# liangheming/simple_pose

Hardware: AMD Instinct MI355X
Metric: images/sec fwd+decode, ResNet50-DConv 256x192 bs=128 (higher is better)
Workload: dtype f32; 1 GPU; ResNet50-DConv 256x192 bs=128 per GPU, fp32 forward (NCHW in -> heat maps) + GaussTaylor decode, eval-mode BN, conditioned random weights; images_per_gpu=128, global_batch=128, parallelism=replicas x1 (no collective), ranks=1 process(es), one per GPU, launch=stream launches, tile_table=profiles/r06_dconv_f32_tiles.json, batches_in_flight=2, decode=in line, HSA_ENABLE_IPC_MODE_LEGACY=0

## Files before the change

include/simple_pose_hip.h:

```cpp
#ifndef SIMPLE_POSE_HIP_H
#define SIMPLE_POSE_HIP_H

#include <stdint.h>

#ifdef __cplusplus
extern "C" {
#endif

#define SP_OK 0
#define SP_EINVAL (-1)
#define SP_ELAUNCH (-2)

#define SP_ABI_VERSION 36

#define SP_CONV_RELU 0x1u
#define SP_CONV_OUT_NCHW 0x2u
#define SP_CONV_PIXEL_SHUFFLE 0x4u
#define SP_CONV_OUT_F32 0x10u
#define SP_CONV_BN_Y_MASK 0x20u
#define SP_CONV_BF16 0x8u
#define SP_CONV_HARDSWISH 0x40u
#define SP_CONV_OUT_SLICE 0x80u

typedef struct sp_conv_desc {
// ... 20 lines not shown
#define SP_CONV_KERNEL_RING_LW 3
#define SP_CONV_KERNEL_RING_LW4 4
#define SP_CONV_KERNEL_PW 2

int sp_abi_version(void);
const char* sp_last_error(void);


int sp_nchw_to_nhwc4(const float* x_nchw, float* y_nhwc4, int batch, int channels, int h, int w, void* stream);

int sp_conv2d_fwd(const sp_conv_desc* desc, const void* x, const void* w_packed, const float* scale,
                  const float* shift, const void* residual, void* y, void* stream);

int sp_conv3x3_direct_ok(const sp_conv_desc* desc);
int sp_conv3x3_direct(const sp_conv_desc* desc, const void* x, const void* w_packed, const float* scale, const float* shift,
                      const void* residual, void* y, void* stream);

int sp_basic_block_c32_ok(const sp_conv_desc* desc);
int sp_basic_block_c32(const sp_conv_desc* desc, const void* x, const void* w1_packed, const float* scale1, const float* shift1,
                       const void* w2_packed, const float* scale2, const float* shift2, void* y, void* stream);

int sp_basic_block_c64_ok(const sp_conv_desc* desc);
int sp_basic_block_c64(const sp_conv_desc* desc, const void* x, const void* w1_packed, const float* scale1, const float* shift1,
                       const void* w2_packed, const float* scale2, const float* shift2, void* y, void* stream);

int sp_dual_pw_bf16_ok(int64_t rows, int c_main, int c_short, int c_out);
int sp_dual_pw_f32_ok(int64_t rows, int c_main, int c_short, int c_out);
int sp_dual_pw_f32(const float* a_main, const float* w_main_packed, const float* scale_main, const float* shift_main, const float* a_short,
                   const float* w_short_packed, const float* scale_short, const float* shift_short, float* y, int64_t rows, int c_main, int c_short,
                   int c_out, int relu, void* stream);
int sp_dual_pw_bf16(const void* a_main, const void* w_main_packed, const float* scale_main, const float* shift_main, const void* a_short,
                    const void* w_short_packed, const float* scale_short, const float* shift_short, void* y, int64_t rows, int c_main, int c_short,
                    int c_out, int relu, void* stream);
int sp_bottleneck_c64_ok(const sp_conv_desc* desc);
int sp_bottleneck_c64(const sp_conv_desc* desc, const void* x, const void* w1_packed, const float* scale1, const float* shift1,
                      const void* w2_packed, const float* scale2, const float* shift2, const void* w3_packed, const float* scale3,
                      const float* shift3, void* y, void* stream);

int sp_stem7_pool_ok(int batch, int h, int w);
int sp_stem7_pool(const float* x, const void* w_packed, int k_pad, const float* scale, const float* shift, void* y, int bf16,
                  int batch, int h, int w, void* stream);
int sp_stem7_pool_u8(const unsigned char* crops_bgr, const float* mean_rgb_host, const void* w_packed, int k_pad, const float* scale,
                     const float* shift, void* y, int bf16, int batch, int h, int w, void* stream);

int sp_hrnet_transition1_ok(int c_in, int h, int w);
int sp_hrnet_transition1(const void* x, int batch, int h, int w, const void* wa_packed, int k_pad, const float* scale_a, const float* shift_a,
                         const void* wb_packed, const float* scale_b, const float* shift_b, void* y_hi, void* y_lo, void* stream);
int sp_hrnet_stem_ok(int batch, int h, int w);
int sp_hrnet_stem(const float* x, const void* w1_packed, int k1_pad, const float* scale1, const float* shift1, const void* w2_packed,
                  const float* scale2, const float* shift2, void* y, int batch, int h, int w, void* stream);

int sp_conv2d_pw_ok(const sp_conv_desc* desc);

int sp_conv2d_ring_ok(const sp_conv_desc* desc);

int sp_conv2d_kernel_name(const sp_conv_desc* desc, int has_residual, int variant, char* buf, int cap);

int sp_conv2d_default_tile(const sp_conv_desc* desc, int* tile_m, int* tile_n);

int sp_maxpool3x3s2_nhwc(const float* x, float* y, int batch, int h, int w, int c, void* stream);

int sp_pixel_shuffle2_nhwc(const float* x, float* y, int batch, int h, int w, int c, void* stream);

int sp_global_avg_pool_nhwc(const float* x, float* y, int batch, int hw, int c, void* stream);
int sp_se_gate_add_relu_nhwc(const float* x, const float* gate_logits, const float* identity, float* y, int batch, int hw,
                             int c, void* stream);
// ... 321 lines not shown
```

simple_pose_amd/_lib.py:

```python
from __future__ import annotations

import ctypes
import os
from ctypes import c_double, c_float, c_int, c_int32, c_int64, c_uint32, c_void_p

from .build import LIB_PATH as _DEFAULT_LIB_PATH

LIB_PATH = os.environ.get("SIMPLE_POSE_HIP_LIB", _DEFAULT_LIB_PATH)

SP_CONV_RELU = 0x1
SP_CONV_OUT_NCHW = 0x2
SP_CONV_PIXEL_SHUFFLE = 0x4
SP_CONV_BF16 = 0x8
SP_CONV_OUT_F32 = 0x10
SP_CONV_BN_Y_MASK = 0x20
SP_CONV_HARDSWISH = 0x40
SP_CONV_OUT_SLICE = 0x80
SP_LETTERBOX_FOCUS, SP_LETTERBOX_U8 = 0, 1
SP_YOLO_NMS_MAX_CANDIDATES, SP_YOLO_NMS_MAX_DET = 32768, 1024
SP_COCO_MAX_JOINTS, SP_COCO_MAX_GT_PER_IMAGE, SP_COCO_MAX_DT_PER_IMAGE, SP_COCO_MAX_DETS = 64, 128, 2048, 32
SP_COCO_DT_XY_F64, SP_COCO_DT_SCORE_F64, SP_COCO_GT_CROWD, SP_COCO_GT_IGNORE = 1, 2, 1, 2
CONV_TILES =((128, 128), (64, 128), (128, 64), (64, 64), (256, 64), (128, 32))
ABI_VERSION = 36
SP_CONV_KERNEL_IGEMM, SP_CONV_KERNEL_RING, SP_CONV_KERNEL_PW, SP_CONV_KERNEL_RING_LW, SP_CONV_KERNEL_RING_LW4 = 0, 1, 2, 3, 4
# ... 116 lines not shown
    "sp_coco_kp_accumulate": (c_int, [_P, _P, _P, _P, _P, c_int, c_int, c_int, c_int, c_int, ctypes.POINTER(c_double), c_int, _P, c_int64, _P, _P, _P]),
    "sp_pixel_unshuffle2_nhwc": (c_int, [_P, _P, c_int, c_int, c_int, c_int, _P]),
    "sp_pixel_unshuffle2_nhwc_bf16": (c_int, [_P, _P, c_int, c_int, c_int, c_int, _P]),
    "sp_maxpool3x3s2_idx_nhwc": (c_int, [_P, c_int, _P, _P, c_int, c_int, c_int, c_int, _P]),
    "sp_maxpool3x3s2_bwd_idx_nhwc": (c_int, [_P, _P, c_int, _P, c_int, c_int, c_int, c_int, _P]),
    "sp_nchw_to_nhwc_pad": (c_int, [_P, _P, c_int, c_int, c_int, c_int, c_int, c_int, _P]),
    "sp_warp_affine_u8c3": (c_int, [_P, c_int, c_int, _P, c_int, _P, c_int, c_int, _P]),
    "sp_warp_affine_batch_u8c3_to_nchw_f32": (c_int, [_P, _P, _P, _P, c_int, c_int, c_int, ctypes.POINTER(c_float), _P, _P, _P]),
    "sp_conv2d_bn_stats_rows": (c_int, [ctypes.POINTER(ConvDesc), ctypes.POINTER(c_int)]),
    "sp_conv2d_fwd_bn_stats": (c_int, [ctypes.POINTER(ConvDesc), _P, _P, _P, _P, _P, c_int, _P]),
    "sp_conv2d_fwd_bn_stats_abn": (c_int, [ctypes.POINTER(ConvDesc), _P, _P, _P, _P, _P, _P, _P, _P, _P, _P, _P, c_int, _P]),
    "sp_bn_train_stats_from_conv": (c_int, [_P, _P, c_int, c_int, c_int64, c_int, c_float, c_float, _P, _P, _P, _P, _P]),
    "sp_conv2d_dgrad_bn_bwd_stats": (c_int, [ctypes.POINTER(ConvDesc), _P, _P, _P, _P, _P, _P, _P, _P, _P, _P, c_int, _P]),
    "sp_conv2d_dgrad_bn_bwd_stats2": (c_int, [ctypes.POINTER(ConvDesc), _P, _P, _P, _P, _P, _P, _P, _P, _P, _P, _P, _P, _P, _P, c_int, _P]),
    "sp_conv2d_dgrad_bn_bwd_stats_macc": (c_int, [ctypes.POINTER(ConvDesc), _P, _P, _P, _P, _P, _P, _P, _P, _P, _P, _P, _P, _P, _P, _P, c_int, _P]),
    "sp_conv2d_dgrad_phases": (c_int, [ctypes.POINTER(ConvDesc), c_int, _P, ctypes.POINTER(_P), _P, _P, _P, _P, _P, _P, _P, _P, _P, _P, _P, _P, c_int, _P]),
    "sp_bn_sums_from_conv": (c_int, [_P, _P, c_int, c_int, c_int, _P, _P]),
    "sp_bn_fold_apply_nhwc": (c_int, [_P, c_int, _P, _P, c_int, c_int, c_int64, c_float, c_float, _P, _P, _P, _P, c_int64, c_int, c_int, _P, _P, _P, _P, _P, _P]),
    "sp_bn_fold_bwd_apply_nhwc": (c_int, [_P, c_int, _P, _P, _P, _P, _P, c_int, c_int, _P, _P, _P, c_int64, c_int64, c_int, _P, _P, _P, _P, _P, _P, c_int, _P]),
    "sp_bn_bwd_sums_from_conv": (c_int, [_P, _P, c_int, c_int, c_int, _P, _P, _P]),
    "sp_bn_bwd_sums_from_conv_pair": (c_int, [_P, _P, _P, c_int, c_int, c_int, _P, _P, _P, _P, _P]),
    "sp_u8hwc_bgr_to_nhwc": (c_int, [_P, _P, c_int, c_int, c_int, c_int, _P, _P]),
    "sp_nchw_to_nhwc4_bf16": (c_int, [_P, _P, c_int, c_int, c_int, c_int, _P]),
    "sp_conv3x3_direct_ok": (c_int, [ctypes.POINTER(ConvDesc)]),
    "sp_conv3x3_direct": (c_int, [ctypes.POINTER(ConvDesc), _P, _P, _P, _P, _P, _P, _P]),
    "sp_basic_block_c32_ok": (c_int, [ctypes.POINTER(ConvDesc)]),
    "sp_basic_block_c32": (c_int, [ctypes.POINTER(ConvDesc), _P, _P, _P, _P, _P, _P, _P, _P, _P]),
    "sp_basic_block_c64_ok": (c_int, [ctypes.POINTER(ConvDesc)]),
    "sp_basic_block_c64": (c_int, [ctypes.POINTER(ConvDesc), _P, _P, _P, _P, _P, _P, _P, _P, _P]),
    "sp_dual_pw_bf16_ok": (c_int, [c_int64, c_int, c_int, c_int]),
    "sp_dual_pw_f32_ok": (c_int, [c_int64, c_int, c_int, c_int]),
    "sp_dual_pw_f32": (c_int, [_P, _P, _P, _P, _P, _P, _P, _P, _P, c_int64, c_int, c_int, c_int, c_int, _P]),
    "sp_dual_pw_bf16": (c_int, [_P, _P, _P, _P, _P, _P, _P, _P, _P, c_int64, c_int, c_int, c_int, c_int, _P]),
    "sp_bottleneck_c64_ok": (c_int, [ctypes.POINTER(ConvDesc)]),
    "sp_conv2d_pw_ok": (c_int, [ctypes.POINTER(ConvDesc)]),
    "sp_hrnet_stem_ok": (c_int, [c_int, c_int, c_int]),
    "sp_hrnet_stem": (c_int, [_P, _P, c_int, _P, _P, _P, _P, _P, _P, c_int, c_int, c_int, _P]),
    "sp_hrnet_transition1_ok": (c_int, [c_int, c_int, c_int]),
    "sp_hrnet_transition1": (c_int, [_P, c_int, c_int, c_int, _P, c_int, _P, _P, _P, _P, _P, _P, _P, _P]),
    "sp_stem7_pool_ok": (c_int, [c_int, c_int, c_int]),
    "sp_stem7_pool": (c_int, [_P, _P, c_int, _P, _P, _P, c_int, c_int, c_int, c_int, _P]),
    "sp_stem7_pool_u8": (c_int, [_P, ctypes.POINTER(ctypes.c_float), _P, c_int, _P, _P, _P, c_int, c_int, c_int, c_int, _P]),
    "sp_bottleneck_c64": (c_int, [ctypes.POINTER(ConvDesc), _P, _P, _P, _P, _P, _P, _P, _P, _P, _P, _P, _P]),
    "sp_masked_mse": (c_int, [_P, _P, _P, c_int, c_int, c_int, _P, _P, _P, _P]),
    "sp_conv_packed_dims": (c_int, [c_int, c_int, c_int, ctypes.POINTER(c_int), ctypes.POINTER(c_int)]),
    "sp_pack_conv_weights": (c_int, [_P, c_int, c_int, c_int, c_int, c_int, c_int, c_int, c_int, c_int, c_int, _P, c_int, _P]),
    "sp_pack_conv_weights_grouped": (c_int, [_P, c_int, c_int, c_int, c_int, c_int, _P, c_int, _P]),
    "sp_pack_conv_weights_grouped_taps": (c_int, [_P, c_int, c_int, c_int, c_int, c_int, c_int, c_int, c_int, c_int, c_int, c_int, c_int, _P, c_int, _P]),
    "sp_conv2d_wgrad_grouped_workspace": (c_int, [c_int, c_int, c_int, c_int, c_int, c_int, ctypes.POINTER(c_int64)]),
    "sp_conv2d_wgrad_grouped": (c_int, [_P, _P, c_int, c_int, c_int, c_int, c_int, c_int, c_int, c_int, c_int, c_int, c_int, c_int, _P, _P, c_int64, _P]),
    "sp_pack_deconv_k4s2p1": (c_int, [_P, c_int, c_int, c_int, _P, c_int, _P]),
    "sp_fold_bn": (c_int, [_P, _P, _P, _P, c_int, c_float, c_int, _P, _P, _P]),
    "sp_yolo_letterbox": (c_int, [_P, c_int, c_int, c_int, c_int, c_int, c_int, c_int, c_int, c_int, c_int, _P, _P]),
    "sp_yolo_focus_nchw": (c_int, [_P, c_int, c_int, c_int, _P, _P]),
    "sp_yolo_spp_nhwc": (c_int, [_P, c_int, c_int, c_int, c_int, c_int, _P]),
    "sp_upsample2_slice_nhwc": (c_int, [_P, c_int, _P, c_int, c_int, c_int, c_int, c_int, _P]),
    "sp_yolo_head_decode": (c_int, [_P, _P, _P, c_int, ctypes.POINTER(c_int32), c_int, c_int, c_int, ctypes.POINTER(c_float), ctypes.POINTER(c_float), _P, _P]),
    "sp_yolo_nms_workspace": (c_int, [c_int, ctypes.POINTER(c_int64)]),
    "sp_yolo_nms": (c_int, [_P, c_int, c_int, c_int, c_float, c_float, c_int, c_int, c_int, c_int, _P, c_int64, _P, ctypes.POINTER(c_int32), ctypes.POINTER(c_int32), _P]),
    "sp_yolo_boxes_to_source": (c_int, [_P, c_int, c_float, c_float, c_float, c_float, c_float, _P]),
    "sp_yolo_nms_device": (c_int, [_P, c_int, c_int, c_int, c_float, c_float, c_int, c_int, c_int, c_int, _P, c_int64, _P, _P, _P, _P]),
    "sp_topdown_plan": (c_int, [_P, _P, c_int, c_int, c_int, c_float, c_int, c_int, c_int, c_int, c_int, _P, _P, _P, _P, _P, _P, _P, _P, _P, _P, _P]),
    "sp_warp_affine_plan_u8c3": (c_int, [_P, c_int, c_int, c_int, _P, _P, _P, c_int, _P, c_int, c_int, _P]),
    "sp_mirror_w": (c_int, [_P, _P, c_int64, c_int, c_int, _P]),
    "sp_heat_map_flip_merge": (c_int, [_P, _P, ctypes.POINTER(c_int32), c_int, c_int, c_int, c_int, c_int, _P, _P]),
    "sp_track_associate": (c_int, [_P, _P, _P, _P, _P, _P, c_int, c_int, ctypes.POINTER(c_double), c_double, c_int, c_int, _P, _P, _P, _P, _P, _P, _P, _P,
# ... 102 lines not shown
```

simple_pose_amd/csrc/conv_pw.hip:

```cpp
#include "sp_common.h"

namespace {

struct PwArgs {
    const float* x;
    const float* w;
    const float* scale;
    const float* shift;
    const float* res;
    float* y;
    int M, N, nchunks, tiles_m, relu;
    unsigned x_bytes, y_bytes;
};

constexpr int BM = 64;
constexpr int TRS = 68;
constexpr unsigned OOB = 0x80000000u;

template <int K>
__global__ __launch_bounds__(256, 1) void conv_pw_kernel(const PwArgs p) {
    constexpr int CH = K / 4;
    constexpr int NG = K / 8;
    constexpr int APT = BM * CH / 256;
    extern __shared__ __align__(16) float smem[];
// ... 210 lines not shown
                    for (int i = 0; i < 2; ++i) fa[(g + 1) & 1][i] = *reinterpret_cast<const f32x4*>(a + swz(i * 32 + fr, 2 * (g + 1) + fh));
                }
#pragma unroll
                for (int s = 0; s < 4; ++s)
#pragma unroll
                    for (int i = 0; i < 2; ++i)
#pragma unroll
                        for (int n = 0; n < 2; ++n)
                            acc[q][i][n] = __builtin_amdgcn_mfma_f32_32x32x2f32(fa[g & 1][i][s], fb[q][g][n][s], acc[q][i][n], 0, 0, 0);
            }
        }
#pragma unroll
        for (int i = 0; i < 2; ++i)
#pragma unroll
            for (int n = 0; n < 2; ++n)
#pragma unroll
                for (int r = 0; r < 16; ++r) {
                    const float vd = acc[1][i][n][r] * sdv[n] + hdv[n];
                    float v = acc[0][i][n][r] * s3v[n] + h3v[n];
                    v += vd;
                    if (p.relu) v = v > 0.f ? v : 0.f;
                    tr[(i * 32 + (r & 3) + 8 * (r >> 2) + 4 * fh) * TRS + n * 32 + fr] = v;
                }
#pragma unroll
        for (int it = 0; it < 16; ++it) {
            const int row = m0 + it * 4 + rsub;
            const unsigned off = row < p.M ? (unsigned)(((size_t)row * p.N + nbase + c4) * 4) : OOB;
            const f32x4 v = *reinterpret_cast<const f32x4*>(tr + (it * 4 + rsub) * TRS + c4);
            __builtin_amdgcn_raw_buffer_store_b128(__builtin_bit_cast(u32x4, v), yr, off, 0, 0);
        }
        if (more) park_a(cur ^ 1);
        __syncthreads();
    }
}

template <int K>
int launch_pw_dual(const PwDualArgs& a, hipStream_t stream) {
    constexpr int lds = (4 * BM * K + 4 * BM * TRS) * 4;
    if (sp_reserve_lds<&conv_pw_dual_kernel<K>>(lds, "conv_pw_dual")) return SP_ELAUNCH;
    int slots = sp_device_cus() / a.nchunks;
    if (slots < 1) slots = 1;
    if (slots > a.tiles_m) slots = a.tiles_m;
    const int rounds = (a.tiles_m + slots - 1) / slots;
    slots = (a.tiles_m + rounds - 1) / rounds;
    hipLaunchKernelGGL(conv_pw_dual_kernel<K>, dim3(slots * a.nchunks), dim3(256), lds, stream, a);
    return sp_check_launch("conv_pw_dual_kernel");
}

template <int K>
int launch_pw(const PwArgs& a, hipStream_t stream) {
    constexpr int lds = (2 * BM * K + 4 * BM * TRS) * 4;
    if (sp_reserve_lds<&conv_pw_kernel<K>>(lds, "conv_pw")) return SP_ELAUNCH;
    int slots = sp_device_cus() / a.nchunks;
    if (slots < 1) slots = 1;
    if (slots > a.tiles_m) slots = a.tiles_m;
    const int rounds = (a.tiles_m + slots - 1) / slots;
    slots = (a.tiles_m + rounds - 1) / rounds;
    hipLaunchKernelGGL(conv_pw_kernel<K>, dim3(slots * a.nchunks), dim3(256), lds, stream, a);
    return sp_check_launch("conv_pw_kernel");
}

}

extern "C" int sp_conv2d_pw_ok(const sp_conv_desc* d) {
    if (d && d->c_in_group > 0) return 0;
    if (!d) return 0;
// ... 14 lines not shown
    PwArgs a;
    a.x = reinterpret_cast<const float*>(x); a.w = reinterpret_cast<const float*>(w_packed); a.scale = scale; a.shift = shift;
    a.res = reinterpret_cast<const float*>(residual); a.y = reinterpret_cast<float*>(y);
    a.M = (int)M; a.N = d->c_out; a.nchunks = d->c_out / 256; a.tiles_m = (int)((M + BM - 1) / BM);
    a.relu = (d->flags & SP_CONV_RELU) ? 1 : 0;
    a.x_bytes = (unsigned)(M * d->c_in * 4); a.y_bytes = (unsigned)(M * d->c_out * 4);
    if (sp_name_query_active()) {
        sp_name_query_set("conv_pw_kernel<%d>", d->c_in);
        return SP_OK;
    }
    return d->c_in == 64 ? launch_pw<64>(a, (hipStream_t)stream) : launch_pw<128>(a, (hipStream_t)stream);
}


extern "C" int sp_dual_pw_f32_ok(int64_t rows, int c_main, int c_short, int c_out) {
    return rows > 0 && rows * (int64_t)c_out < (1ll << 30) && c_main == 64 && c_short == 64 && c_out > 0 && c_out % 256 == 0;
}

extern "C" int sp_dual_pw_f32(const float* a_main, const float* w_main_packed, const float* scale_main, const float* shift_main, const float* a_short,
                              const float* w_short_packed, const float* scale_short, const float* shift_short, float* y, int64_t rows, int c_main,
                              int c_short, int c_out, int relu, void* stream) {
    SP_REQUIRE(a_main && w_main_packed && a_short && w_short_packed && y, "sp_dual_pw_f32: null pointer");
    SP_REQUIRE(sp_dual_pw_f32_ok(rows, c_main, c_short, c_out), "sp_dual_pw_f32: two fp32 1x1 stride-1 products of 64 channels each into a multiple of 256 (got %d + %d -> %d, %lld rows)",
               c_main, c_short, c_out, (long long)rows);
    SP_REQUIRE(y != a_main && y != a_short, "sp_dual_pw_f32: y must not alias an input");
    if (sp_name_query_active()) { sp_name_query_set("conv_pw_dual_kernel<64>"); return SP_OK; }
    PwDualArgs a;
    a.x_main = a_main; a.x_short = a_short; a.w_main = w_main_packed; a.w_short = w_short_packed;
    a.s_main = scale_main; a.h_main = shift_main; a.s_short = scale_short; a.h_short = shift_short; a.y = y;
    a.M = (int)rows; a.N = c_out; a.nchunks = c_out / 256; a.tiles_m = (int)((rows + BM - 1) / BM); a.relu = relu ? 1 : 0;
    a.x_bytes = (unsigned)(rows * 64 * 4); a.y_bytes = (unsigned)(rows * c_out * 4);
    return launch_pw_dual<64>(a, (hipStream_t)stream);
}
```

simple_pose_amd/engine.py:

```python
from __future__ import annotations

import ctypes
import os

from dataclasses import dataclass, field
from typing import Dict, List, Optional, Tuple

import torch

from . import _lib, conv_geometry
from ._lib import ConvDesc, SP_CONV_BF16, SP_CONV_HARDSWISH, SP_CONV_OUT_NCHW, SP_CONV_OUT_SLICE, SP_CONV_PIXEL_SHUFFLE, SP_CONV_RELU
from .conv_geometry import n_pad_for, round_up as _round_up

BN_EPS = 1e-5


class HipPacker:

    @staticmethod
    def _dims(c_out: int, k: int, bf16: bool) -> Tuple[int, int]:
        n_pad, k_pad = ctypes.c_int(0), ctypes.c_int(0)
        _lib.check(_lib.lib().sp_conv_packed_dims(c_out, k, int(bf16), ctypes.byref(n_pad), ctypes.byref(k_pad)), "sp_conv_packed_dims")
        return n_pad.value, k_pad.value

# ... 152 lines not shown
        for i, op in enumerate(self.ops):
            tails[op.lane] = i
        self._sync[key] = (waits, set(records), tails)
        return self._sync[key]

    def _lane_streams(self, key, n_lanes: int, device=None) -> list:
        pool = self._streams.setdefault(str(key), [])
        while len(pool) < n_lanes - 1:
            pool.append(torch.cuda.Stream(device=device if device is not None else key))
        return pool

    def _launch(self, lib, op: Op, bufs, B: int, stream) -> None:
        P = _lib.ptr
        if op.kind == "conv":
            op.desc.batch = B
            fn = lib.sp_conv3x3_direct if op.direct else lib.sp_conv2d_fwd
            _lib.check(fn(op.desc, P(bufs[op.src]), P(op.w), P(op.scale), P(op.shift),
                          P(bufs[op.res]) if op.res else None, P(bufs[op.dst]) + 4 * op.c0, stream), op.name)
        elif op.kind in ("bb32", "bb64"):
            op.desc.batch = B
            w2, scale2, shift2 = op.args
            _lib.check((lib.sp_basic_block_c32 if op.kind == "bb32" else lib.sp_basic_block_c64)(op.desc, P(bufs[op.src]), P(op.w), P(op.scale), P(op.shift), P(w2), P(scale2), P(shift2),
                                              P(bufs[op.dst]), stream), op.name)
        elif op.kind == "bneck64":
            op.desc.batch = B
            w1, s1, h1, w3, s3, h3 = op.args
            _lib.check(lib.sp_bottleneck_c64(op.desc, P(bufs[op.src]), P(w1), P(s1), P(h1), P(op.w), P(op.scale), P(op.shift), P(w3), P(s3), P(h3),
                                             P(bufs[op.dst]), stream), op.name)
        elif op.kind == "dual1x1":
            w_s, s_s, h_s, rows_per_image, relu = op.args
            fn = lib.sp_dual_pw_bf16 if op.w.element_size() == 2 else lib.sp_dual_pw_f32
            _lib.check(fn(P(bufs[op.src]), P(op.w), P(op.scale), P(op.shift), P(bufs[op.res]), P(w_s), P(s_s), P(h_s), P(bufs[op.dst]),
                                           B * rows_per_image, 64, 64, 256, relu, stream), op.name)
        elif op.kind == "stem7":
            h, w, k_pad, unfused = op.args
            src = bufs[op.src]
            if src.dtype == torch.uint8:
                mean = (ctypes.c_float * 3)(0.485, 0.456, 0.406)
                _lib.check(lib.sp_stem7_pool_u8(P(src), mean, P(op.w), k_pad, P(op.scale), P(op.shift), P(bufs[op.dst]), int(self.dtype == "bf16"),
                                                B, h, w, stream), op.name)
            else:
                _lib.check(lib.sp_stem7_pool(P(src), P(op.w), k_pad, P(op.scale), P(op.shift), P(bufs[op.dst]), int(self.dtype == "bf16"),
                                             B, h, w, stream), op.name)
        elif op.kind == "htrans":
            h, w, k_pad, wb, sb, hb, _ = op.args
            _lib.check(lib.sp_hrnet_transition1(P(bufs[op.src]), B, h, w, P(op.w), k_pad, P(op.scale), P(op.shift), P(wb), P(sb), P(hb),
                                                P(bufs[op.dst]), P(bufs[op.dst2]), stream), op.name)
        elif op.kind == "hstem":
            h, w, k1_pad, w2, s2, h2, unfused = op.args
            src = bufs[op.src]
            if src.dtype == torch.uint8:
                tmp = dict(bufs)
                for u in unfused[:-1]:
                    uh, uw, uc = self.shapes[u.dst]
                    tmp[u.dst] = torch.empty(B * uh * uw * uc, dtype=torch.bfloat16, device=src.device)
                for u in unfused:
                    self._launch(lib, u, tmp, B, stream)
            else:
                _lib.check(lib.sp_hrnet_stem(P(src), P(op.w), k1_pad, P(op.scale), P(op.shift), P(w2), P(s2), P(h2), P(bufs[op.dst]), B, h, w,
                                             stream), op.name)
        elif op.kind == "maxpool":
            h, w, c = op.args
            fn = lib.sp_maxpool3x3s2_nhwc_bf16 if self.dtype == "bf16" else lib.sp_maxpool3x3s2_nhwc
            _lib.check(fn(P(bufs[op.src]), P(bufs[op.dst]), B, h, w, c, stream), op.name)
        elif op.kind == "to_nhwc4":
            c, h, w = op.args
# ... 423 lines not shown
            if self.decoder is not None:
                out = self.decoder(out, trans_inv)
            if self._done[k] is None:
                self._done[k] = torch.cuda.Event()
            self._done[k].record(st)
        return out

    def sync(self) -> None:
        for ev in self._done:
            if ev is not None:
                torch.cuda.current_stream().wait_event(ev)

    def close(self) -> None:
        torch.cuda.synchronize()
        mine = range(self._slot0, self._slot0 + self.depth)
        for key in [k for k in self.prog._pools if len(k) == 3 and k[2] in mine]:
            del self.prog._pools[key]
        for table in (self.prog._streams, self.prog._events):
            for key in [k for k in table if "/" in k and k.rsplit("/", 1)[1].isdigit() and int(k.rsplit("/", 1)[1]) in mine]:
                del table[key]
        self._hm = [None] * self.depth


class ProgramBuilder:

    def __init__(self, in_h: int, in_w: int, dtype: str = "fp32", packer=None):
        if dtype not in ("fp32", "bf16"):
            raise ValueError(dtype)
        self.packer = packer or HipPacker()
        self.fuse_blocks = False
        self.fuse_blocks64 = False
        self.fuse_bottlenecks = False
        self.fuse_tail = os.environ.get("SP_FUSE_TAIL", "1") != "0"
        self.fuse_stem = True
        self.fuse_terms = True
        self.fuse_transition = True
        self.p = Program(dtype=dtype)
        self.bf16 = dtype == "bf16"
        self.cpad = 8 if self.bf16 else 4
        self.p.shapes["input"] = (in_h, in_w, 3)
        self._n = 0
        self.lane = 0

    def _add(self, op: Op) -> None:
        op.lane = self.lane
        self.p.ops.append(op)

    def _fresh(self, stem: str) -> str:
        self._n += 1
        return f"{stem}#{self._n}"

    def to_nhwc4(self, src: str) -> str:
        h, w, c = self.p.shapes[src]
        dst = self._fresh("x4")
        self.p.shapes[dst] = (h, w, 4)
        self._add(Op("to_nhwc4", src, dst, args=(c, h, w), name="to_nhwc4"))
        return dst

    def stem_pool(self, src: str, weight: torch.Tensor, scale, shift, name: str = "conv1") -> str:
        first = len(self.p.ops)
        x4 = self.to_nhwc4(src)
        y = self.conv(x4, weight, stride=2, pad=3, scale=scale, shift=shift, relu=True, name=name)
        out = self.maxpool(y)
        h, w, _ = self.p.shapes[src]
        if not (self.fuse_stem and tuple(weight.shape) == (64, 3, 7, 7) and _lib.lib().sp_stem7_pool_ok(1, h, w)):
            return out
# ... 218 lines not shown
        y = b.dual_pointwise_tail(t, sd[p + ".conv3.weight"], s3, h3, x, sd[p + ".downsample.0.weight"], sdn, hdn, name=p + ".conv3+downsample")
        if y is not None:
            return y
    if (p + ".downsample.0.weight") in sd:
        sdn, hdn = _bn(b, sd, p + ".downsample.1")
        idn = b.conv(x, sd[p + ".downsample.0.weight"], stride=stride, scale=sdn, shift=hdn, name=p + ".downsample")
    s3, h3 = _bn(b, sd, p + ".bn3")
    if (p + ".se.fc.0.weight") in sd:
        z = b.conv(t, sd[p + ".conv3.weight"], scale=s3, shift=h3, name=p + ".conv3")
        g = b.gap(z)
        g = b.conv(g, sd[p + ".se.fc.0.weight"], shift=b.packer.bias(sd[p + ".se.fc.0.bias"]), relu=True, name=p + ".se.fc.0")
        g = b.conv(g, sd[p + ".se.fc.2.weight"], shift=b.packer.bias(sd[p + ".se.fc.2.bias"]), name=p + ".se.fc.2")
        return b.se_gate(z, g, idn)
    return b.conv(t, sd[p + ".conv3.weight"], scale=s3, shift=h3, relu=True, res=idn, name=p + ".conv3")


def _res_basic_block(b: ProgramBuilder, sd, x: str, p: str, stride: int) -> str:
    s1, h1 = _bn(b, sd, p + ".bn1")
    t = b.conv(x, sd[p + ".conv1.weight"], stride=stride, pad=1, scale=s1, shift=h1, relu=True, name=p + ".conv1")
    idn = x
    if (p + ".downsample.0.weight") in sd:
        sdn, hdn = _bn(b, sd, p + ".downsample.1")
        idn = b.conv(x, sd[p + ".downsample.0.weight"], stride=stride, scale=sdn, shift=hdn, name=p + ".downsample")
    s2, h2 = _bn(b, sd, p + ".bn2")
    if (p + ".se.fc.0.weight") in sd:
        z = b.conv(t, sd[p + ".conv2.weight"], pad=1, scale=s2, shift=h2, name=p + ".conv2")
        g = b.gap(z)
        g = b.conv(g, sd[p + ".se.fc.0.weight"], shift=b.packer.bias(sd[p + ".se.fc.0.bias"]), relu=True, name=p + ".se.fc.0")
        g = b.conv(g, sd[p + ".se.fc.2.weight"], shift=b.packer.bias(sd[p + ".se.fc.2.bias"]), name=p + ".se.fc.2")
        return b.se_gate(z, g, idn)
    return b.conv(t, sd[p + ".conv2.weight"], pad=1, scale=s2, shift=h2, relu=True, res=idn, name=p + ".conv2")


def resnet_program(sd: Dict[str, torch.Tensor], head: str, in_h: int = 256, in_w: int = 192,
                   blocks=(3, 4, 6, 3), dtype: str = "fp32", packer=None, fuse_bottlenecks: bool = False, fuse_stem: bool = True) -> Program:
    b = ProgramBuilder(in_h, in_w, dtype, packer)
    b.fuse_bottlenecks = fuse_bottlenecks
    b.fuse_tail = fuse_bottlenecks and b.fuse_tail
    b.fuse_stem = fuse_stem
    s, h = _bn(b, sd, "bn1")
    x = b.stem_pool("input", sd["conv1.weight"], s, h, name="conv1")
    basic = "layer1.0.conv3.weight" not in sd
    for li, n in enumerate(blocks, start=1):
        for bi in range(n):
            x = (_res_basic_block if basic else _bottleneck)(b, sd, x, f"layer{li}.{bi}", 2 if (bi == 0 and li > 1) else 1)
    J = sd["final_layer.weight"].shape[0]
    if head == "dconv":
        for idx in (0, 3, 6):
            s, h = _bn(b, sd, f"deconv_layers.{idx + 1}")
            x = b.deconv_k4s2p1(x, sd[f"deconv_layers.{idx}.weight"], scale=s, shift=h, relu=True,
                                name=f"deconv_layers.{idx}")
        b.conv(x, sd["final_layer.weight"], shift=b.packer.bias(sd["final_layer.bias"]), out_nchw=True,
               dst="heat", name="final_layer")
    elif head == "duc":
        x = b.pixel_shuffle(x)
        for idx in (1, 2):
            s, h = _bn(b, sd, f"duc_layers.{idx}.bn", pixel_shuffle=True)
            x = b.conv(x, sd[f"duc_layers.{idx}.conv.weight"], pad=1, scale=s, shift=h, relu=True, pixel_shuffle=True,
                       name=f"duc_layers.{idx}")
        b.conv(x, sd["final_layer.weight"], pad=1, shift=b.packer.bias(sd["final_layer.bias"]), out_nchw=True,
               dst="heat", name="final_layer")
    else:
        raise ValueError(head)
    hh, ww, _ = b.p.shapes["heat"]
    b.p.out_shape = (J, hh, ww)
    return b.p


def _basic_block(b: ProgramBuilder, sd, x: str, p: str) -> str:
    s1, h1 = _bn(b, sd, p + ".bn1")
    s2, h2 = _bn(b, sd, p + ".bn2")
    fused = b.basic_block_c32(x, sd[p + ".conv1.weight"], s1, h1, sd[p + ".conv2.weight"], s2, h2, name=p)
    if fused is not None:
        return fused
    t = b.conv(x, sd[p + ".conv1.weight"], pad=1, scale=s1, shift=h1, relu=True, name=p + ".conv1")
    return b.conv(t, sd[p + ".conv2.weight"], pad=1, scale=s2, shift=h2, relu=True, res=x, name=p + ".conv2")


# ... 246 lines not shown
```

simple_pose_amd/nets/_resnet_base.py:

```python
from __future__ import annotations

from typing import Optional

import torch
from torch import nn

from .. import engine
from .._lib import HipLibraryError, require_cuda_f32
from ..metrics.flip import COCO_JOINT_PAIRS, merge_flipped, mirror_input, pairs_to_perm


class _Bottleneck(nn.Module):
    expansion = 4

    def __init__(self, inplanes: int, planes: int, stride: int, with_downsample: bool, with_se: bool = False, width: int = 0, groups: int = 1):
        super().__init__()
        width = width or planes
        self.conv1 = nn.Conv2d(inplanes, width, 1, bias=False)
        self.bn1 = nn.BatchNorm2d(width)
        self.conv2 = nn.Conv2d(width, width, 3, stride=stride, padding=1, groups=groups, bias=False)
        self.bn2 = nn.BatchNorm2d(width)
        self.conv3 = nn.Conv2d(width, planes * 4, 1, bias=False)
        self.bn3 = nn.BatchNorm2d(planes * 4)
        if with_downsample:
# ... 50 lines not shown
        inplanes = 64
        Block = _Bottleneck if block == "bottleneck" else _BasicBlock
        for li, (planes, n) in enumerate(zip((64, 128, 256, 512), self.BLOCKS), start=1):
            blocks = []
            for bi in range(n):
                stride = 2 if (bi == 0 and li > 1) else 1
                down = bi == 0 and (stride != 1 or inplanes != planes * Block.expansion)
                blocks.append(Block(inplanes, planes, stride, with_downsample=down, with_se=(reduction and down),
                                    width=planes * width_per_group // 64 * groups, groups=groups))
                inplanes = planes * Block.expansion
            setattr(self, f"layer{li}", nn.Sequential(*blocks))
        self._build_head(inplanes, num_classes)
        self._init_like_reference()
        self.compute_dtype = "fp32"
        self.autotune = True
        self._program: Optional[engine.Program] = None
        self._program_key = None

    def _init_like_reference(self):
        for m in self.modules():
            if isinstance(m, (nn.Conv2d, nn.ConvTranspose2d)):
                nn.init.normal_(m.weight, std=0.001)
                if m.bias is not None:
                    nn.init.constant_(m.bias, 0)
            elif isinstance(m, nn.BatchNorm2d):
                nn.init.constant_(m.weight, 1)
                nn.init.constant_(m.bias, 0)

    def _build_head(self, inplanes: int, num_classes: int):
        raise NotImplementedError

    fuse_bottlenecks = True
    fuse_stem = True

    def _tensors_key(self, x):
        sd = self.state_dict(keep_vars=True)
        return (tuple(x.shape[2:]), str(x.device), self.compute_dtype, self.fuse_bottlenecks, self.fuse_stem) + tuple((v.data_ptr(), v._version) for v in sd.values())

    def hip_program(self, x: torch.Tensor) -> engine.Program:
        key = self._tensors_key(x)
        if self._program is None or key != self._program_key:
            sd = {k: v.detach() for k, v in self.state_dict(keep_vars=True).items()}
            for k, v in sd.items():
                if v.device != x.device:
                    raise HipLibraryError(f"parameter {k} is on {v.device} but the input is on {x.device}; call .to(device)")
            self._program = engine.resnet_program(sd, self.HEAD, in_h=x.shape[2], in_w=x.shape[3], blocks=self.BLOCKS,
                                                   dtype=self.compute_dtype, fuse_bottlenecks=self.fuse_bottlenecks, fuse_stem=self.fuse_stem)
            self._program_key = key
        return self._program

    def forward(self, x: torch.Tensor) -> torch.Tensor:
        x = require_cuda_f32(x, "input")
        if x.dim() != 4 or x.shape[1] != 3 or x.shape[2] % 32 or x.shape[3] % 32:
            raise ValueError(f"expected [B,3,H,W] with H,W multiples of 32, got {tuple(x.shape)}")
        if self.training:
            return self._forward_train(x)
        prog = self.hip_program(x)
        if self.autotune and x.shape[0] >= 16 and x.shape[0] >= 4 * prog.tuned_for_batch:
            prog.autotune(x)
        return prog.run(x)

    def _forward_train(self, x: torch.Tensor) -> torch.Tensor:
        return train_forward(self, x)

    def forward_crops(self, crops: torch.Tensor, flip_test: bool = False, joint_pairs=COCO_JOINT_PAIRS, shift_heatmap: bool = False) -> torch.Tensor:
        return forward_uint8_crops(self, crops, flip_test, joint_pairs, shift_heatmap)


def train_forward(self, x: torch.Tensor) -> torch.Tensor:
    from ..train import PoseTrainer
    import torch.distributed as dist
    if dist.is_available() and dist.is_initialized() and dist.get_world_size() > 1 and not getattr(self, "_warned_local_bn", False):
        import warnings
        warnings.warn("simple_pose_amd: model(x) in train() mode under an initialised process group uses per-rank BatchNorm statistics "
                      "(sync_bn: False behaviour); PoseTrainer(model, process_group=..., sync_bn=True).step() is the SyncBatchNorm path")
        self._warned_local_bn = True
    key = (x.shape[2], x.shape[3], str(x.device), self.compute_dtype)
    tr = getattr(self, "_trainer", None)
    if tr is None or self._trainer_key != key or not tr.still_owns_parameters():
        tr = PoseTrainer(self, in_h=x.shape[2], in_w=x.shape[3], dtype="bf16" if self.compute_dtype == "bf16" else "fp32",
# ... 55 lines not shown
```

Before: 11320 images/s.

## Fuse bottleneck conv3 with next block's conv1 into one fp32 pointwise chain kernel

Adds a persistent HIP kernel that computes a 64->256 pointwise conv with BN, residual add and ReLU. It keeps the resulting tile in LDS and immediately applies the next block's 256->64/128 pointwise conv with BN and ReLU. A program pass replaces matching conv3/conv1 op pairs in fp32 ResNet bottleneck programs. The aim is to avoid re-reading the 256-channel activation from global memory and to save a launch. It costs high LDS use and one block per CU, which limits occupancy.

Measured after the change: 11450 images/s, median of 6. 1.01x the previous value.

```diff
diff --git a/include/simple_pose_hip.h b/include/simple_pose_hip.h
--- a/include/simple_pose_hip.h
+++ b/include/simple_pose_hip.h
@@ -76,6 +76,10 @@
 int sp_dual_pw_bf16(const void* a_main, const void* w_main_packed, const float* scale_main, const float* shift_main, const void* a_short,
                     const void* w_short_packed, const float* scale_short, const float* shift_short, void* y, int64_t rows, int c_main, int c_short,
                     int c_out, int relu, void* stream);
+int sp_pw_chain_f32_ok(int64_t rows, int c_mid, int c_out, int c_next);
+int sp_pw_chain_f32(const float* t, const float* w3_packed, const float* scale3, const float* shift3, const float* residual, float* y,
+                    const float* w1_packed, const float* scale1, const float* shift1, float* t_next, int64_t rows, int c_mid, int c_out, int c_next,
+                    void* stream);
 int sp_bottleneck_c64_ok(const sp_conv_desc* desc);
 int sp_bottleneck_c64(const sp_conv_desc* desc, const void* x, const void* w1_packed, const float* scale1, const float* shift1,
                       const void* w2_packed, const float* scale2, const float* shift2, const void* w3_packed, const float* scale3,
diff --git a/simple_pose_amd/_lib.py b/simple_pose_amd/_lib.py
--- a/simple_pose_amd/_lib.py
+++ b/simple_pose_amd/_lib.py
@@ -172,6 +172,8 @@
     "sp_dual_pw_f32_ok": (c_int, [c_int64, c_int, c_int, c_int]),
     "sp_dual_pw_f32": (c_int, [_P, _P, _P, _P, _P, _P, _P, _P, _P, c_int64, c_int, c_int, c_int, c_int, _P]),
     "sp_dual_pw_bf16": (c_int, [_P, _P, _P, _P, _P, _P, _P, _P, _P, c_int64, c_int, c_int, c_int, c_int, _P]),
+    "sp_pw_chain_f32_ok": (c_int, [c_int64, c_int, c_int, c_int]),
+    "sp_pw_chain_f32": (c_int, [_P, _P, _P, _P, _P, _P, _P, _P, _P, _P, c_int64, c_int, c_int, c_int, _P]),
     "sp_bottleneck_c64_ok": (c_int, [ctypes.POINTER(ConvDesc)]),
     "sp_conv2d_pw_ok": (c_int, [ctypes.POINTER(ConvDesc)]),
     "sp_hrnet_stem_ok": (c_int, [c_int, c_int, c_int]),
diff --git a/simple_pose_amd/csrc/conv_pw.hip b/simple_pose_amd/csrc/conv_pw.hip
--- a/simple_pose_amd/csrc/conv_pw.hip
+++ b/simple_pose_amd/csrc/conv_pw.hip
@@ -266,6 +266,210 @@
         if (more) park_a(cur ^ 1);
         __syncthreads();
     }
+}
+
+struct PwChainArgs {
+    const float* x;
+    const float* w;
+    const float* scale;
+    const float* shift;
+    const float* res;
+    float* y;
+    const float* w1;
+    const float* scale1;
+    const float* shift1;
+    float* t;
+    int M, tiles_m;
+    unsigned x_bytes, y_bytes, t_bytes;
+};
+
+constexpr int T2S = 36;
+
+template <int K, int NEXT>
+__global__ __launch_bounds__(256, 1) void conv_pw_chain_kernel(const PwChainArgs p) {
+    static_assert(K == 64 && (NEXT == 64 || NEXT == 128), "conv3 of a 64-channel Bottleneck into a 64- or 128-channel conv1");
+    constexpr int N = 256;
+    constexpr int CH = K / 4;
+    constexpr int NG = K / 8;
+    constexpr int NG1 = N / 8;
+    constexpr int APT = BM * CH / 256;
+    constexpr int RT = NEXT / 64;
+    extern __shared__ __align__(16) float smem[];
+    float* const As = smem;
+    const int tid = threadIdx.x, lane = tid & 63, wave = tid >> 6;
+    float* const ys = smem + 2 * BM * K;
+    float* const tr = ys + wave * (BM * TRS);
+    float* const t2 = ys + 4 * BM * TRS + wave * (RT * 32 * T2S);
+    const int fr = lane & 31, fh = lane >> 5;
+    const int slot = blockIdx.x, nslots = gridDim.x;
+    const int nbase = wave * 64;
+    const int cn = NEXT == 64 ? wave >> 1 : wave;
+    const int ri0 = NEXT == 64 ? wave & 1 : 0;
+
+    const __amdgpu_buffer_rsrc_t xr = __builtin_amdgcn_make_buffer_rsrc(const_cast<float*>(p.x), (short)0, p.x_bytes, 0x00020000);
+    const __amdgpu_buffer_rsrc_t yr = __builtin_amdgcn_make_buffer_rsrc(p.y, (short)0, p.y_bytes, 0x00020000);
+    const __amdgpu_buffer_rsrc_t rr = __builtin_amdgcn_make_buffer_rsrc(const_cast<float*>(p.res), (short)0, p.y_bytes, 0x00020000);
+    const __amdgpu_buffer_rsrc_t tnr = __builtin_amdgcn_make_buffer_rsrc(p.t, (short)0, p.t_bytes, 0x00020000);
+
+    float fb[NG][2][4];
+#pragma unroll
+    for (int g = 0; g < NG; ++g)
+#pragma unroll
+        for (int n = 0; n < 2; ++n) {
+            const f32x4 t = *reinterpret_cast<const f32x4*>(p.w + (size_t)(nbase + n * 32 + fr) * K + 8 * g + 4 * fh);
+            fb[g][n][0] = t[0]; fb[g][n][1] = t[1]; fb[g][n][2] = t[2]; fb[g][n][3] = t[3];
+        }
+    float fw[NG1][4];
+#pragma unroll
+    for (int g = 0; g < NG1; ++g) {
+        const f32x4 t = *reinterpret_cast<const f32x4*>(p.w1 + (size_t)(cn * 32 + fr) * N + 8 * g + 4 * fh);
+        fw[g][0] = t[0]; fw[g][1] = t[1]; fw[g][2] = t[2]; fw[g][3] = t[3];
+    }
+    const int c4 = (lane & 15) * 4, rsub = lane >> 4;
+    f32x4 sc4 = {1.f, 1.f, 1.f, 1.f}, sh4 = {0.f, 0.f, 0.f, 0.f};
+    if (p.scale) sc4 = *reinterpret_cast<const f32x4*>(p.scale + nbase + c4);
+    if (p.shift) sh4 = *reinterpret_cast<const f32x4*>(p.shift + nbase + c4);
+    const float s1v = p.scale1 ? p.scale1[cn * 32 + fr] : 1.f, h1v = p.shift1 ? p.shift1[cn * 32 + fr] : 0.f;
+
+    auto swz = [](int row, int chunk) { return row * K + ((chunk ^ (row & (CH - 1))) << 2); };
+    u32x4 sa[APT];
+    auto load_a = [&](int mt) {
+        const unsigned base = (unsigned)mt * (BM * K * 4);
+#pragma unroll
+        for (int i = 0; i < APT; ++i) sa[i] = __builtin_amdgcn_raw_buffer_load_b128(xr, base + (unsigned)((tid + 256 * i) * 16), 0, 0);
+    };
+    auto park_a = [&](int buf) {
+#pragma unroll
+        for (int i = 0; i < APT; ++i) {
+            const int q = tid + 256 * i;
+            *reinterpret_cast<u32x4*>(As + buf * (BM * K) + swz(q / CH, q % CH)) = sa[i];
+        }
+    };
+    unsigned off[16];
+    u32x4 rv[16];
+    auto load_res = [&](int mt) {
+#pragma unroll
+        for (int it = 0; it < 16; ++it) {
+            const int row = mt * BM + it * 4 + rsub;
+            off[it] = row < p.M ? (unsigned)(((size_t)row * N + nbase + c4) * 4) : OOB;
+        }
+#pragma unroll
+        for (int it = 0; it < 16; ++it) rv[it] = __builtin_amdgcn_raw_buffer_load_b128(rr, off[it], 0, 0);
+    };
+
+    int mt = slot;
+    if (mt >= p.tiles_m) return;
+    load_a(mt);
+    park_a(0);
+    load_res(mt);
+    __syncthreads();
+    int cur = 0;
+    for (; mt < p.tiles_m; mt += nslots, cur ^= 1) {
+        const int m0 = mt * BM;
+        const bool more = mt + nslots < p.tiles_m;
+        if (more) load_a(mt + nslots);
+
+        f32x16 acc[2][2];
+#pragma unroll
+        for (int i = 0; i < 2; ++i)
+#pragma unroll
+            for (int n = 0; n < 2; ++n)
+#pragma unroll
+                for (int r = 0; r < 16; ++r) acc[i][n][r] = 0.f;
+        const float* a = As + cur * (BM * K);
+        f32x4 fa[2][2];
+#pragma unroll
+        for (int i = 0; i < 2; ++i) fa[0][i] = *reinterpret_cast<const f32x4*>(a + swz(i * 32 + fr, fh));
+#pragma unroll
+        for (int g = 0; g < NG; ++g) {
+            if (g + 1 < NG) {
+#pragma unroll
+                for (int i = 0; i < 2; ++i) fa[(g + 1) & 1][i] = *reinterpret_cast<const f32x4*>(a + swz(i * 32 + fr, 2 * (g + 1) + fh));
+            }
+#pragma unroll
+            for (int s = 0; s < 4; ++s)
+#pragma unroll
+                for (int i = 0; i < 2; ++i)
+#pragma unroll
+                    for (int n = 0; n < 2; ++n)
+                        acc[i][n] = __builtin_amdgcn_mfma_f32_32x32x2f32(fa[g & 1][i][s], fb[g][n][s], acc[i][n], 0, 0, 0);
+        }
+
+#pragma unroll
+        for (int i = 0; i < 2; ++i)
+#pragma unroll
+            for (int n = 0; n < 2; ++n)
+#pragma unroll
+                for (int r = 0; r < 16; ++r) tr[(i * 32 + (r & 3) + 8 * (r >> 2) + 4 * fh) * TRS + n * 32 + fr] = acc[i][n][r];
+#pragma unroll
+        for (int it = 0; it < 16; ++it) {
+            f32x4* const slot4 = reinterpret_cast<f32x4*>(tr + (it * 4 + rsub) * TRS + c4);
+            f32x4 v = *slot4;
+#pragma unroll
+            for (int e = 0; e < 4; ++e) v[e] = v[e] * sc4[e] + sh4[e];
+            const f32x4 r4 = __builtin_bit_cast(f32x4, rv[it]);
+#pragma unroll
+            for (int e = 0; e < 4; ++e) v[e] += r4[e];
+#pragma unroll
+            for (int e = 0; e < 4; ++e) v[e] = v[e] > 0.f ? v[e] : 0.f;
+            __builtin_amdgcn_raw_buffer_store_b128(__builtin_bit_cast(u32x4, v), yr, off[it], 0, 0);
+            *slot4 = v;
+        }
+        if (more) park_a(cur ^ 1);
+        __syncthreads();
+        if (more) load_res(mt + nslots);
+
+        f32x16 c[RT];
+#pragma unroll
+        for (int i = 0; i < RT; ++i)
+#pragma unroll
+            for (int r = 0; r < 16; ++r) c[i][r] = 0.f;
+        auto yfrag = [&](int i, int g) { return *reinterpret_cast<const f32x4*>(ys + (g >> 3) * (BM * TRS) + ((ri0 + i) * 32 + fr) * TRS + 8 * (g & 7) + 4 * fh); };
+        f32x4 fy[2][RT];
+#pragma unroll
+        for (int i = 0; i < RT; ++i) fy[0][i] = yfrag(i, 0);
+#pragma unroll
+        for (int g = 0; g < NG1; ++g) {
+            if (g + 1 < NG1) {
+#pragma unroll
+                for (int i = 0; i < RT; ++i) fy[(g + 1) & 1][i] = yfrag(i, g + 1);
+            }
+#pragma unroll
+            for (int s = 0; s < 4; ++s)
+#pragma unroll
+                for (int i = 0; i < RT; ++i) c[i] = __builtin_amdgcn_mfma_f32_32x32x2f32(fy[g & 1][i][s], fw[g][s], c[i], 0, 0, 0);
+        }
+#pragma unroll
+        for (int i = 0; i < RT; ++i)
+#pragma unroll
+            for (int r = 0; r < 16; ++r) {
+                float v = c[i][r] * s1v + h1v;
+                v = v > 0.f ? v : 0.f;
+                t2[(i * 32 + (r & 3) + 8 * (r >> 2) + 4 * fh) * T2S + fr] = v;
+            }
+#pragma unroll
+        for (int it = 0; it < RT * 4; ++it) {
+            const int lr = it * 8 + (lane >> 3), cc = (lane & 7) * 4;
+            const int row = m0 + ri0 * 32 + lr;
+            const unsigned o = row < p.M ? (unsigned)(((size_t)row * NEXT + cn * 32 + cc) * 4) : OOB;
+            const f32x4 v = *reinterpret_cast<const f32x4*>(t2 + lr * T2S + cc);
+            __builtin_amdgcn_raw_buffer_store_b128(__builtin_bit_cast(u32x4, v), tnr, o, 0, 0);
+        }
+        __syncthreads();
+    }
+}
+
+template <int NEXT>
+int launch_pw_chain(const PwChainArgs& a, hipStream_t stream) {
+    constexpr int lds = (2 * BM * 64 + 4 * BM * TRS + 4 * (NEXT / 64) * 32 * T2S) * 4;
+    if (sp_reserve_lds<&conv_pw_chain_kernel<64, NEXT>>(lds, "conv_pw_chain")) return SP_ELAUNCH;
+    int slots = sp_device_cus();
+    if (slots < 1) slots = 1;
+    if (slots > a.tiles_m) slots = a.tiles_m;
+    const int rounds = (a.tiles_m + slots - 1) / slots;
+    slots = (a.tiles_m + rounds - 1) / rounds;
+    hipLaunchKernelGGL((conv_pw_chain_kernel<64, NEXT>), dim3(slots), dim3(256), lds, stream, a);
+    return sp_check_launch("conv_pw_chain_kernel");
 }
 
 template <int K>
@@ -346,3 +550,24 @@
     a.x_bytes = (unsigned)(rows * 64 * 4); a.y_bytes = (unsigned)(rows * c_out * 4);
     return launch_pw_dual<64>(a, (hipStream_t)stream);
 }
+
+extern "C" int sp_pw_chain_f32_ok(int64_t rows, int c_mid, int c_out, int c_next) {
+    return rows > 0 && rows * (int64_t)c_out <= (1ll << 29) && c_mid == 64 && c_out == 256 && (c_next == 64 || c_next == 128);
+}
+
+extern "C" int sp_pw_chain_f32(const float* t, const float* w3_packed, const float* scale3, const float* shift3, const float* residual, float* y,
+                               const float* w1_packed, const float* scale1, const float* shift1, float* t_next, int64_t rows, int c_mid, int c_out,
+                               int c_next, void* stream) {
+    SP_REQUIRE(t && w3_packed && residual && y && w1_packed && t_next, "sp_pw_chain_f32: null pointer");
+    SP_REQUIRE(sp_pw_chain_f32_ok(rows, c_mid, c_out, c_next),
+               "sp_pw_chain_f32: an fp32 1x1 product 64 -> 256 chained into a 1x1 product 256 -> 64 or 128 (got %d -> %d -> %d, %lld rows)", c_mid, c_out,
+               c_next, (long long)rows);
+    SP_REQUIRE(y != t && y != residual && t_next != t && t_next != residual && t_next != y, "sp_pw_chain_f32: y and t_next must not alias an input or each other");
+    if (sp_name_query_active()) { sp_name_query_set("conv_pw_chain_kernel<64, %d>", c_next); return SP_OK; }
+    PwChainArgs a;
+    a.x = t; a.w = w3_packed; a.scale = scale3; a.shift = shift3; a.res = residual; a.y = y;
+    a.w1 = w1_packed; a.scale1 = scale1; a.shift1 = shift1; a.t = t_next;
+    a.M = (int)rows; a.tiles_m = (int)((rows + BM - 1) / BM);
+    a.x_bytes = (unsigned)(rows * 64 * 4); a.y_bytes = (unsigned)(rows * 256 * 4); a.t_bytes = (unsigned)(rows * c_next * 4);
+    return c_next == 64 ? launch_pw_chain<64>(a, (hipStream_t)stream) : launch_pw_chain<128>(a, (hipStream_t)stream);
+}
diff --git a/simple_pose_amd/engine.py b/simple_pose_amd/engine.py
--- a/simple_pose_amd/engine.py
+++ b/simple_pose_amd/engine.py
@@ -208,6 +208,10 @@
             fn = lib.sp_dual_pw_bf16 if op.w.element_size() == 2 else lib.sp_dual_pw_f32
             _lib.check(fn(P(bufs[op.src]), P(op.w), P(op.scale), P(op.shift), P(bufs[op.res]), P(w_s), P(s_s), P(h_s), P(bufs[op.dst]),
                                            B * rows_per_image, 64, 64, 256, relu, stream), op.name)
+        elif op.kind == "pwchain":
+            w1, s1, h1, rows_per_image, c_next, _ = op.args
+            _lib.check(lib.sp_pw_chain_f32(P(bufs[op.src]), P(op.w), P(op.scale), P(op.shift), P(bufs[op.res]), P(bufs[op.dst]), P(w1), P(s1), P(h1),
+                                           P(bufs[op.dst2]), B * rows_per_image, 64, 256, c_next, stream), op.name)
         elif op.kind == "stem7":
             h, w, k_pad, unfused = op.args
             src = bufs[op.src]
@@ -697,6 +701,7 @@
         self.fuse_blocks64 = False
         self.fuse_bottlenecks = False
         self.fuse_tail = os.environ.get("SP_FUSE_TAIL", "1") != "0"
+        self.fuse_chain = os.environ.get("SP_FUSE_CHAIN", "1") != "0"
         self.fuse_stem = True
         self.fuse_terms = True
         self.fuse_transition = True
@@ -981,8 +986,41 @@
     return b.conv(t, sd[p + ".conv2.weight"], pad=1, scale=s2, shift=h2, relu=True, res=idn, name=p + ".conv2")
 
 
+def _plain_pointwise(d) -> bool:
+    return (d.c_in_group == 0 and d.taps_h == 1 and d.taps_w == 1 and d.stride == 1 and d.stride_x in (0, 1) and d.phases_y == 1 and d.phases_x == 1 and
+            d.dy0 == 0 and d.dx0 == 0 and (d.grid_h, d.grid_w) == (d.in_h, d.in_w) == (d.out_h, d.out_w) and d.oy_mul == 1 and d.ox_mul == 1 and
+            d.oy_add == 0 and d.ox_add == 0 and d.k_pad == d.c_in and d.n_pad == d.c_out and d.out_c == d.c_out)
+
+
+def _fuse_pw_chains(b: "ProgramBuilder", sd) -> None:
+    if b.bf16 or not b.fuse_chain:
+        return
+    ops, out, i = b.p.ops, [], 0
+    while i < len(ops):
+        a, c = ops[i], ops[i + 1] if i + 1 < len(ops) else None
+        ok = (c is not None and a.kind == "conv" and c.kind == "conv" and a.lane == c.lane and a.name.endswith(".conv3") and c.name.endswith(".conv1") and
+              a.res is not None and c.res is None and c.src == a.dst and not a.direct and not c.direct and a.c0 == 0 and c.c0 == 0 and
+              a.scale is not None and a.shift is not None and c.scale is not None and c.shift is not None)
+        if ok:
+            blk, da, dc = a.name[:-len(".conv3")], a.desc, c.desc
+            ok = ((blk + ".downsample.0.weight") not in sd and (blk + ".se.fc.0.weight") not in sd and _plain_pointwise(da) and _plain_pointwise(dc) and
+                  da.flags == SP_CONV_RELU and dc.flags == SP_CONV_RELU and da.c_in == 64 and da.c_out == 256 and dc.c_in == 256 and
+                  dc.c_out in (64, 128) and tuple(a.w.shape) == (256, 64) and tuple(c.w.shape) == (dc.c_out, 256) and
+                  _lib.lib().sp_pw_chain_f32_ok(da.grid_h * da.grid_w, 64, 256, dc.c_out))
+        if ok:
+            out.append(Op("pwchain", a.src, a.dst, res=a.res, dst2=c.dst, w=a.w, scale=a.scale, shift=a.shift,
+                          args=(c.w, c.scale, c.shift, da.grid_h * da.grid_w, dc.c_out, (a, c)), name=a.name + "+" + c.name, flops=a.flops + c.flops,
+                          lane=a.lane))
+            i += 2
+        else:
+            out.append(a)
+            i += 1
+    b.p.ops[:] = out
+
+
 def resnet_program(sd: Dict[str, torch.Tensor], head: str, in_h: int = 256, in_w: int = 192,
-                   blocks=(3, 4, 6, 3), dtype: str = "fp32", packer=None, fuse_bottlenecks: bool = False, fuse_stem: bool = True) -> Program:
+                   blocks=(3, 4, 6, 3), dtype: str = "fp32", packer=None, fuse_bottlenecks: bool = False, fuse_stem: bool = True,
+                   fuse_chain: bool = False) -> Program:
     b = ProgramBuilder(in_h, in_w, dtype, packer)
     b.fuse_bottlenecks = fuse_bottlenecks
     b.fuse_tail = fuse_bottlenecks and b.fuse_tail
@@ -993,6 +1031,8 @@
     for li, n in enumerate(blocks, start=1):
         for bi in range(n):
             x = (_res_basic_block if basic else _bottleneck)(b, sd, x, f"layer{li}.{bi}", 2 if (bi == 0 and li > 1) else 1)
+    if fuse_chain and not basic:
+        _fuse_pw_chains(b, sd)
     J = sd["final_layer.weight"].shape[0]
     if head == "dconv":
         for idx in (0, 3, 6):
diff --git a/simple_pose_amd/nets/_resnet_base.py b/simple_pose_amd/nets/_resnet_base.py
--- a/simple_pose_amd/nets/_resnet_base.py
+++ b/simple_pose_amd/nets/_resnet_base.py
@@ -106,10 +106,11 @@
 
     fuse_bottlenecks = True
     fuse_stem = True
+    fuse_chain = True
 
     def _tensors_key(self, x):
         sd = self.state_dict(keep_vars=True)
-        return (tuple(x.shape[2:]), str(x.device), self.compute_dtype, self.fuse_bottlenecks, self.fuse_stem) + tuple((v.data_ptr(), v._version) for v in sd.values())
+        return (tuple(x.shape[2:]), str(x.device), self.compute_dtype, self.fuse_bottlenecks, self.fuse_stem, self.fuse_chain) + tuple((v.data_ptr(), v._version) for v in sd.values())
 
     def hip_program(self, x: torch.Tensor) -> engine.Program:
         key = self._tensors_key(x)
@@ -119,7 +120,8 @@
                 if v.device != x.device:
                     raise HipLibraryError(f"parameter {k} is on {v.device} but the input is on {x.device}; call .to(device)")
             self._program = engine.resnet_program(sd, self.HEAD, in_h=x.shape[2], in_w=x.shape[3], blocks=self.BLOCKS,
-                                                   dtype=self.compute_dtype, fuse_bottlenecks=self.fuse_bottlenecks, fuse_stem=self.fuse_stem)
+                                                   dtype=self.compute_dtype, fuse_bottlenecks=self.fuse_bottlenecks, fuse_stem=self.fuse_stem,
+                                                   fuse_chain=self.fuse_chain)
             self._program_key = key
         return self._program
 
```
